# roclark/torchsr

Measured on AMD Instinct MI355X. Metric: 96x96 HR crops/sec (SRGAN GAN train step), higher is better.
Workload: dtype f32; 1 GPU; SRGAN full GAN step (Generator + Discriminator + VGG19 perceptual loss), 96x96 HR crops, batch 16 per GPU, fp32; per_gpu_batch=16, global_batch=16, crop=96, parallelism=dp1, hip_graph=True, vgg19_weights=seeded-random, plan_cus=256

## Files before the change

### include/srx.h

```cpp
#ifndef SRX_H
#define SRX_H

#include <stddef.h>
#include <stdint.h>

#ifdef __cplusplus
extern "C" {
#endif

#define SRX_VERSION 100

enum {
  SRX_OK = 0,
  SRX_E_BADARG = 1,
  SRX_E_UNSUPPORTED = 2,
  SRX_E_HIP = 3,
  SRX_E_WORKSPACE = 4
};

enum { SRX_ACT_NONE = 0, SRX_ACT_RELU = 1, SRX_ACT_LRELU = 2, SRX_ACT_PRELU = 3 };

int srx_version(void);
int srx_last_error(char* buf, size_t n);
int srx_build_info(char* buf, size_t n);
// ... 237 lines not shown
int srx_l1_fwd_count(const float* a, const float* b, float* loss, int64_t n, int64_t count, float* ws, void* stream);
int srx_l1_bwd_count(const float* a, const float* b, const float* gscale, float* da, float* db, int64_t n, int64_t count,
                     void* stream);
int srx_bce_fwd(const float* p, float target, float* loss, int64_t n, float* ws, void* stream);
int srx_bce_bwd(const float* p, float target, const float* gscale, float* dp, int64_t n, void* stream);
int srx_bce_logits_fwd(const float* x, const float* shift, float target, float* loss, int64_t n, float* ws, void* stream);
int srx_bce_logits_bwd(const float* x, const float* shift, float target, const float* gscale, float* dx, int64_t n, void* stream);
int srx_mean_fwd(const float* x, float* out, int64_t n, float* ws, void* stream);
int srx_mean_bwd(const float* x, const float* gscale, float* dx, int64_t n, void* stream);

enum { SRX_HEAD_SRGAN_D = 0, SRX_HEAD_SRGAN_G = 1, SRX_HEAD_ESRGAN_D = 2, SRX_HEAD_ESRGAN_G = 3 };
typedef struct {
  int32_t mode, B, J, n_first;
  float slope, adv_weight;
} srx_gan_head_t;
int srx_gan_head_fwd(const srx_gan_head_t* h, const float* hidden, const float* w2, const float* b2, const float* shift,
                     const float* addend, float* zp, float* out, float* loss, void* stream);
int srx_gan_head_bwd(const srx_gan_head_t* h, const float* hidden, const float* w2, const float* zp, const float* out,
                     const float* shift, const float* g, float* dpre, float* dw2, float* db2, float* db1, int accumulate,
                     void* stream);

int srx_adam_step(float* p, const float* g, float* m, float* v, int64_t n, const float* lr, float beta1,
                  float beta2, float eps, float grad_scale, int64_t* step, void* stream);

#ifdef __cplusplus
}
#endif
#endif
```

### torchsr_amd/_lib.py

```python
import ctypes as C
import os
import subprocess
import sys

_HERE = os.path.dirname(os.path.abspath(__file__))
CSRC = os.path.join(_HERE, 'csrc')
LIB_PATH = os.environ.get('SRX_LIB') or os.path.join(CSRC, 'libsrx_hip.so')
SOURCES = ['api.cpp', 'gconv.hip', 'wgrad.hip', 'convpack.hip', 'c64.hip', 'thin9.hip', 'rdb.hip', 'thin.hip', 'rowtile.hip', 'augment.hip', 'norm.hip', 'eltwise.hip', 'linear.hip', 'loss.hip', 'head.hip', 'wino.hip', 'optim.hip']
HEADERS = ['srx_common.h', 'conv_host.h', os.path.join('..', '..', 'include', 'srx.h')]

ACT_NONE, ACT_RELU, ACT_LRELU, ACT_PRELU = 0, 1, 2, 3


class Conv2dDesc(C.Structure):
    _fields_ = [
        ('N', C.c_int32), ('H', C.c_int32), ('W', C.c_int32),
        ('Cin', C.c_int32), ('Cin_s', C.c_int32), ('Cout', C.c_int32), ('Cout_s', C.c_int32),
        ('KH', C.c_int32), ('KW', C.c_int32), ('stride', C.c_int32), ('pad', C.c_int32),
        ('shuffle', C.c_int32), ('act', C.c_int32), ('slope', C.c_float), ('up', C.c_int32),
        ('precision', C.c_int32),
    ]


class DgradEpilogue(C.Structure):
# ... 220 lines not shown
    'srx_wino_ws_floats': (_Z, [_D, _I]),
    'srx_wino_plan': (_I, [_D, _I, C.POINTER(C.c_int)]),
    'srx_wino_pack': (_I, [_D, _P, _P, _I, _P]),
    'srx_wino_fwd': (_I, [_D, _P, _P, _P, _P, _P, _Z, _P]),
    'srx_wino_bwd_data': (_I, [_D, _P, _P, _P, _P, _P, _Z, _P]),
    'srx_conv3x3_bf16s_applicable': (_I, [_D]),
    'srx_conv3x3_bf16s_packed_bytes': (_Z, [_D]),
    'srx_conv3x3_bf16s_pack': (_I, [_D, _P, _P, _P, _P]),
    'srx_conv3x3_bf16s_ws_floats': (_Z, [_D, _I]),
    'srx_conv3x3_bf16s_fwd': (_I, [_D, _P, _P, _P, _I, _P, _I, _P, _Z, _P]),
    'srx_conv3x3_bf16s_bwd_data': (_I, [_D, _P, _P, _P, _P, _I, _P, _Z, _P]),
    'srx_conv2d_fwd_first3_to_bf16': (_I, [_D, _P, _P, _P, _P, _P]),
    'srx_maxpool2x2_fwd_to_bf16': (_I, [_P, _P, _I, _I, _I, _I, _P]),
    'srx_maxpool2x2_relu_bwd_bf16': (_I, [_P, _P, _P, _I, _I, _I, _I, _P]),
    'srx_act_bwd_from_out_to_bf16': (_I, [_P, _P, _P, C.c_int64, _I, C.c_float, _P]),
    'srx_wino_infer_applicable': (_I, [_D]),
    'srx_wino_fwd_act': (_I, [_D, _P, _P, _P, _P, _P, _P, _Z, _P]),
    'srx_wino_force_plan': (_I, [_I, _I, _I]),
    'srx_wino_stat_rows': (_I, [_D]),
    'srx_wino_fwd_stats': (_I, [_D, _P, _P, _P, _P, _P, _P, _Z, _P]),
    'srx_gan_head_fwd': (_I, [C.POINTER(GanHead), _P, _P, _P, _P, _P, _P, _P, _P, _P]),
    'srx_gan_head_bwd': (_I, [C.POINTER(GanHead), _P, _P, _P, _P, _P, _P, _P, _P, _P, _P, _I, _P]),
    'srx_adam_step': (_I, [_P, _P, _P, _P, _L, _P, _F, _F, _F, _F, _P, _P]),
}
_UNCHECKED = {'srx_wino_applicable', 'srx_wino_infer_applicable', 'srx_conv3x3_bf16s_applicable', 'srx_wino_stat_rows', 'srx_conv2d_bwd_data_bn_rows', 'srx_conv2d_fwd_bn_in_ok', 'srx_conv2d_bwd_data_bn_in_ok', 'srx_pack_table_bytes', 'srx_version', 'srx_last_error', 'srx_device_cus', 'srx_plan_cus', 'srx_prof_stop', 'srx_conv2d_stat_rows', 'srx_bn_stat_rows', 'srx_bn_rows_per_block'}

EXPORTS = tuple(_SIGS.keys())

_lib = None


def load_handle(path: str) -> C.CDLL:
    import torch
    if torch.cuda.is_available():
        torch.cuda.init()
    return C.CDLL(path)


def _ensure_fresh():
    want = source_digest()
    if built_digest(LIB_PATH) == want:
        return
    import fcntl
    with open(os.path.join(CSRC, '.build.lock'), 'w') as lock:
        fcntl.flock(lock, fcntl.LOCK_EX)
        if built_digest(LIB_PATH) == want:
# ... 47 lines not shown
```

### torchsr_amd/csrc/linear.hip

```cpp
#include "srx_common.h"
#include <algorithm>

namespace {

template <int NB>
__global__ __launch_bounds__(256) void linear_fwd_kernel(const float* __restrict__ x, const float* __restrict__ w,
                                                         float* __restrict__ part, int B, int K, int J, int b0,
                                                         int kper) {
  __shared__ f32x4 red[4][64];
  const int tid = threadIdx.x, lane = tid & 63, wave = tid >> 6;
  const int r = lane & 15, h = lane >> 4;
  const int j0 = blockIdx.x * 16;
  const int kbeg = blockIdx.y * kper, kend = min(K, kbeg + kper);
  const int j = j0 + r;
  const bool jok = j < J;
  const float* wr = w + (size_t)(jok ? j : 0) * K;
  const float* xr[NB];
  bool bok[NB];
  f32x4 acc[NB];
#pragma unroll
  for (int n = 0; n < NB; ++n) {
    const int b = b0 + 16 * n + r;
    bok[n] = b < B;
    xr[n] = x + (size_t)(bok[n] ? b : 0) * K;
// ... 322 lines not shown
  f32x4 prev[4];
  if (accumulate) {
#pragma unroll
    for (int g = 0; g < 4; ++g) prev[g] = *reinterpret_cast<const f32x4*>(dw + (size_t)(j0 + 4 * h + g) * K + kcol);
  }
  for (int bb0 = 0; bb0 < B; bb0 += 32) {
    float av[8];
    f32x4 xf[8];
#pragma unroll
    for (int i = 0; i < 8; ++i) {
      av[i] = srx_bload1(rd, dv, (unsigned)srx_uniform((bb0 + 4 * i) * J * 4));
      xf[i] = srx_bload(rx, xv, (unsigned)srx_uniform((bb0 + 4 * i) * K * 4));
    }
#pragma unroll
    for (int i = 0; i < 8; ++i)
#pragma unroll
      for (int e = 0; e < 4; ++e) acc[e] = __builtin_amdgcn_mfma_f32_16x16x4f32(av[i], xf[i][e], acc[e], 0, 0, 0);
  }
#pragma unroll
  for (int g = 0; g < 4; ++g) {
    f32x4 o = {acc[0][g], acc[1][g], acc[2][g], acc[3][g]};
    if (accumulate) o += prev[g];
    *reinterpret_cast<f32x4*>(dw + (size_t)(j0 + 4 * h + g) * K + kcol) = o;
  }
}

bool linear_fast_ok(int B, int K, int J, bool need_j16) {
  const size_t lim = 0xfffffff0ull;
  return K % 64 == 0 && (!need_j16 || J % 16 == 0) && ((size_t)J + 16) * K * 4 < lim && ((size_t)B + 64) * K * 4 < lim && ((size_t)B + 64) * J * 4 < lim;
}

int fwd_splits(int K, int J, int B) {
  const int64_t tiles = srx_cdiv(J, 16) * srx_cdiv(B, 64);
  int64_t s = srx_cdiv(1024, tiles);
  const int64_t maxs = srx_cdiv(K, 256);
  if (s > maxs) s = maxs;
  if (s < 1) s = 1;
  return (int)s;
}
int bwd_splits(int K, int J, int B) {
  const int64_t blocks = srx_cdiv(K, 256) * srx_cdiv(B, 64);
  int64_t s = srx_cdiv(1024, blocks);
  const int64_t maxs = srx_cdiv(J, 64);
  if (s > maxs) s = maxs;
  if (s < 1) s = 1;
  return (int)s;
// ... 56 lines not shown
    else if (nb == 3) hipLaunchKernelGGL(linear_bwd_data_kernel<3>, grid, dim3(256), 0, st, dy, w, ws, B, K, J, b0, jper);
    else hipLaunchKernelGGL(linear_bwd_data_kernel<4>, grid, dim3(256), 0, st, dy, w, ws, B, K, J, b0, jper);
    SRX_CHECK_LAUNCH("linear_bwd_data_kernel");
  }
  const int64_t n = (int64_t)B * K;
  hipLaunchKernelGGL(sum_slabs_kernel, dim3((unsigned)srx_cdiv(n / 4, 256)), dim3(256), 0, st, ws, nsplit, n, dx);
  SRX_CHECK_LAUNCH("sum_slabs_kernel");
  return SRX_OK;
}

extern "C" int srx_linear_bwd_weight(const float* x, const float* dy, float* dw, int accumulate, int B, int K, int J,
                                     void* stream) {
  SRX_REQUIRE(x && dy && dw && B > 0 && K > 0 && J > 0, "linear_bwd_weight: bad argument");
  SRX_REQUIRE(K % 4 == 0, "linear_bwd_weight: in_features must be a multiple of 4");
  if (linear_fast_ok(B, K, J, true))
    hipLaunchKernelGGL(linear_bwd_weight_fast_kernel, dim3((unsigned)srx_cdiv(K, 256), (unsigned)srx_cdiv(J, 16)), dim3(256),
                       0, srx_stream(stream), x, dy, dw, B, K, J, accumulate);
  else
    hipLaunchKernelGGL(linear_bwd_weight_kernel, dim3((unsigned)srx_cdiv(K, 256), (unsigned)srx_cdiv(J, 16)), dim3(256),
                       0, srx_stream(stream), x, dy, dw, B, K, J, accumulate);
  SRX_CHECK_LAUNCH("linear_bwd_weight_kernel");
  return SRX_OK;
}
```

### torchsr_amd/csrc/optim.hip

```cpp
#include "srx_common.h"

namespace {

__global__ void adam_tick_kernel(int64_t* step) { *step += 1; }

__global__ __launch_bounds__(256) void adam_kernel(float* __restrict__ p, const float* __restrict__ g,
                                                   float* __restrict__ m, float* __restrict__ v, int64_t n,
                                                   const float* __restrict__ lr_ptr, float beta1, float beta2,
                                                   float eps, float gscale, const int64_t* __restrict__ step_ptr) {
  const double t = (double)(*step_ptr);
  const float bc1 = (float)(1.0 - pow((double)beta1, t));
  const float bc2 = (float)(1.0 - pow((double)beta2, t));
  const float step_size = lr_ptr[0] / bc1;
  const float bc2_sqrt = sqrtf(bc2);
  const int64_t n4 = n / 4;
  for (int64_t i = (int64_t)blockIdx.x * blockDim.x + threadIdx.x; i < n4; i += (int64_t)gridDim.x * blockDim.x) {
    f32x4 pv = *reinterpret_cast<const f32x4*>(p + i * 4);
    f32x4 gv = *reinterpret_cast<const f32x4*>(g + i * 4);
    f32x4 mv = *reinterpret_cast<const f32x4*>(m + i * 4);
    f32x4 vv = *reinterpret_cast<const f32x4*>(v + i * 4);
#pragma unroll
    for (int e = 0; e < 4; ++e) {
      const float gg = gv[e] * gscale;
      mv[e] = beta1 * mv[e] + (1.f - beta1) * gg;
      vv[e] = beta2 * vv[e] + (1.f - beta2) * gg * gg;
      const float denom = sqrtf(vv[e]) / bc2_sqrt + eps;
      pv[e] -= step_size * (mv[e] / denom);
    }
    *reinterpret_cast<f32x4*>(p + i * 4) = pv;
    *reinterpret_cast<f32x4*>(m + i * 4) = mv;
    *reinterpret_cast<f32x4*>(v + i * 4) = vv;
  }
  if (blockIdx.x == 0 && threadIdx.x < (n & 3)) {
    const int64_t i = n4 * 4 + threadIdx.x;
    const float gg = g[i] * gscale;
    const float mm = beta1 * m[i] + (1.f - beta1) * gg;
    const float vv = beta2 * v[i] + (1.f - beta2) * gg * gg;
    m[i] = mm;
    v[i] = vv;
    p[i] -= step_size * (mm / (sqrtf(vv) / bc2_sqrt + eps));
  }
}

}

extern "C" int srx_adam_step(float* p, const float* g, float* m, float* v, int64_t n, const float* lr, float beta1,
                             float beta2, float eps, float grad_scale, int64_t* step, void* stream) {
  SRX_REQUIRE(p && g && m && v && lr && step && n > 0, "adam_step: bad argument");
  SRX_REQUIRE(((uintptr_t)p % 16 == 0) && ((uintptr_t)g % 16 == 0) && ((uintptr_t)m % 16 == 0) &&
                  ((uintptr_t)v % 16 == 0),
              "adam_step: buffers must be 16-byte aligned");
  hipStream_t st = srx_stream(stream);
  hipLaunchKernelGGL(adam_tick_kernel, dim3(1), dim3(1), 0, st, step);
  SRX_CHECK_LAUNCH("adam_tick_kernel");
  int64_t blocks = srx_cdiv(n / 4, 256);
  if (blocks > 4096) blocks = 4096;
  if (blocks < 1) blocks = 1;
  hipLaunchKernelGGL(adam_kernel, dim3((unsigned)blocks), dim3(256), 0, st, p, g, m, v, n, lr, beta1, beta2, eps,
                     grad_scale, step);
  SRX_CHECK_LAUNCH("adam_kernel");
  return SRX_OK;
}
```

### torchsr_amd/csrc/srx_common.h

```cpp
#pragma once
#include <hip/hip_runtime.h>
#include <hip/hip_ext.h>
#include <stdint.h>
#include <stddef.h>
#include "../../include/srx.h"

typedef float f32x4 __attribute__((ext_vector_type(4)));
typedef float f32x16 __attribute__((ext_vector_type(16)));

void srx_set_error(const char* fmt, ...);

#define SRX_FAIL(code, ...)      \
  do {                           \
    srx_set_error(__VA_ARGS__);  \
    return (code);               \
  } while (0)

#define SRX_REQUIRE(cond, ...) \
  do {                         \
    if (!(cond)) SRX_FAIL(SRX_E_BADARG, __VA_ARGS__); \
  } while (0)

#define SRX_CHECK_LAUNCH(name)                                                        \
  do {                                                                                \
// ... 51 lines not shown
static inline int64_t srx_roundup(int64_t a, int64_t b) { return srx_cdiv(a, b) * b; }

__device__ __forceinline__ void srx_divmod(int m, int d, float inv_d, int& q, int& r) {
  q = __float2int_rz(__int2float_rn(m) * inv_d);
  r = m - q * d;
  if (r < 0) { q -= 1; r += d; }
  if (r >= d) { q += 1; r -= d; }
}

__device__ __forceinline__ __amdgpu_buffer_rsrc_t srx_rsrc(const void* p, unsigned bytes) {
  return __builtin_amdgcn_make_buffer_rsrc(const_cast<void*>(p), (short)0, (int)bytes, 0x00020000);
}
__device__ __forceinline__ f32x4 srx_bload(__amdgpu_buffer_rsrc_t r, unsigned voff, unsigned soff) {
  return __builtin_bit_cast(f32x4, __builtin_amdgcn_raw_buffer_load_b128(r, (int)voff, (int)soff, 0));
}
__device__ __forceinline__ int srx_uniform(int v) { return __builtin_amdgcn_readfirstlane(v); }

__device__ __forceinline__ float srx_wave_sum(float v) {
#pragma unroll
  for (int o = 32; o > 0; o >>= 1) v += __shfl_xor(v, o, 64);
  return v;
}

__device__ __forceinline__ void srx_wino_pack_one(const float* __restrict__ w, float* __restrict__ upk, int Cout, int Cin,
                                                  int transpose, int64_t idx) {
  const int R = transpose == 1 ? Cin : Cout, K = transpose == 1 ? Cout : Cin;
  const int r = (int)(idx / K), k = (int)(idx - (int64_t)r * K);
  const int rsrc = transpose == 2 ? (r % (Cout / 4)) * 4 + r / (Cout / 4) : r;
  float g[3][3];
#pragma unroll
  for (int i = 0; i < 3; ++i)
#pragma unroll
    for (int j = 0; j < 3; ++j)
      g[i][j] = transpose == 1 ? w[(((size_t)k * Cin + r) * 3 + (2 - i)) * 3 + (2 - j)] : w[(((size_t)rsrc * Cin + k) * 3 + i) * 3 + j];
  float t[4][3];
#pragma unroll
  for (int j = 0; j < 3; ++j) {
    t[0][j] = g[0][j];
    t[1][j] = 0.5f * (g[0][j] + g[1][j] + g[2][j]);
    t[2][j] = 0.5f * (g[0][j] - g[1][j] + g[2][j]);
    t[3][j] = g[2][j];
  }
  const int nch = K / 32, rt = R / 32;
  const int jg = r >> 5, mrow = r & 31, kc = k / 32, kk = k % 32, quad = kk >> 2, e = kk & 3, s = quad >> 1, hh = quad & 1;
#pragma unroll
  for (int i = 0; i < 4; ++i) {
// ... 9 lines not shown
```

### torchsr_amd/ddp.py

```python
from typing import Dict, List, Optional, Sequence, Tuple

import torch
import torch.distributed as dist
from torch import Tensor


class BackwardCuts:

    def __init__(self, names: Sequence[str] = ()):
        self.names = set(names)
        self.pairs: Dict[str, List[Tuple[Tensor, Tensor]]] = {}

    def __call__(self, name: str, t: Tensor) -> Tensor:
        if name not in self.names or not torch.is_grad_enabled() or not t.requires_grad:
            return t
        leaf = t.detach().requires_grad_(True)
        self.pairs.setdefault(name, []).append((t, leaf))
        return leaf

    def pending(self, name: str) -> bool:
        return bool(self.pairs.get(name))

    def resume(self, name: str) -> None:
        pairs = [(t, leaf) for t, leaf in self.pairs.pop(name, []) if leaf.grad is not None]
        if pairs:
            torch.autograd.backward([t for t, _ in pairs], [leaf.grad for _, leaf in pairs])

    def clear(self) -> None:
        self.pairs.clear()


class GradBuckets:

    window_bytes = 8 << 20

    def __init__(self, flat, boundaries: Sequence[str] = (), module: Optional[torch.nn.Module] = None,
                 group: Optional[dist.ProcessGroup] = None, force: bool = False, reserve_cus: int = 0, window_hook=None):
        self.reserve_cus = int(reserve_cus)
        self.window_hook = window_hook
        self._window = False
        self.flat = flat
        self.group = group
        self.world_size = dist.get_world_size(group) if dist.is_initialized() else 1
        self.force = bool(force) and dist.is_initialized()
        cuts = [0]
        if boundaries:
            if module is None:
                raise RuntimeError('GradBuckets: boundaries are parameter names of `module`')
            offs = flat.offsets_by_name(module)
            for name in boundaries:
                if name not in offs:
                    raise RuntimeError(f'GradBuckets: no trainable parameter {name!r}')
                cuts.append(offs[name])
        cuts.append(flat.numel)
        if sorted(cuts) != cuts or len(set(cuts)) != len(cuts):
            raise RuntimeError(f'GradBuckets: boundaries must be distinct and in parameter order, got offsets {cuts}')
        self.slices = [flat.grad[a:b] for a, b in zip(cuts[:-1], cuts[1:])]
        self._work = []
        self.issued = 0
        self.timing = False
        self._marks = []
        self._launched = []

    def __len__(self) -> int:
# ... 107 lines not shown
```

### torchsr_amd/esrgan/trainer.py

```python
import torch

from .. import functional as F
from ..layers import no_weight_grad
from ..srgan.trainer import SRGANTrainer
from .discriminator import Discriminator
from .generator import Generator


class ESRGANTrainer(SRGANTrainer):
    phase_prefix = 'esrgan'
    deep_overlap = False
    generator_cls = Generator
    discriminator_cls = Discriminator
    amp_phases = ('psnr', 'gan')
    gen_tail_bucket = 'upsample1.weight'

    def _initialize_loss(self) -> None:
        super()._initialize_loss()
        self.l1_loss = F.l1_loss
        self.pixel_loss = F.l1_loss
        self.bce_loss = F.bce_with_logits

    def _phase_disc(self) -> None:
        self._phase_disc_gen()
        self._phase_disc_loss()

    def _phase_disc_gen(self) -> None:
        with torch.no_grad():
            low4 = F.to_nhwc(self._static['low_res'], 4)
            self._high4 = F.to_nhwc(self._static['high_res'], 4)
        self.disc_optimizer.zero_grad()
        self._super_res = self.generator.forward_nhwc(low4)

    def _phase_disc_loss(self) -> None:
# ... 23 lines not shown
```

### torchsr_amd/functional.py

```python
import contextlib
from typing import Optional, Tuple

import torch
from torch import Tensor
from torch.autograd import Function

from . import _dev, _lib
from ._lib import (ACT_LRELU, ACT_NONE, ACT_PRELU, ACT_RELU, HEAD_ESRGAN_D, HEAD_ESRGAN_G, HEAD_SRGAN_D, HEAD_SRGAN_G,
                   Conv2dDesc, call)

import ctypes as C


direct_grads = [False]


def _sink(param: Optional[Tensor]) -> Optional[Tensor]:
    if not direct_grads[0] or param is None or not param.requires_grad:
        return None
    g = param.grad
    if g is None or not g.is_cuda or g.dtype != torch.float32 or not g.is_contiguous():
        return None
    return g


cut_hook = [None]


def cut_point(name: str, t: Tensor) -> Tensor:
    hook = cut_hook[0]
    return t if hook is None else hook(name, t)


class WeightGradQueue:
    MAXP = 72

    def __init__(self):
        self.groups = {}
        self.pairs = {}

    def add(self, d: Conv2dDesc, x_ptr: int, dy_ptr: int, sink_ptr: int, bias_ptr, keep, scale: float = 1.0) -> None:
        key = tuple(getattr(d, f) for f, _ in Conv2dDesc._fields_)
        self.groups.setdefault(key, [d, []])[1].append((x_ptr, dy_ptr, sink_ptr, bias_ptr or 0, keep, float(scale)))

    def add_pair(self, d: Conv2dDesc, cin_lo: int, x_ptr: int, dy_ptr: int, sinks, bias_sinks, keep) -> None:
        key = ('pair', cin_lo, bias_sinks is None) + tuple(getattr(d, f) for f, _ in Conv2dDesc._fields_)
# ... 1269 lines not shown
        ctx.cfg = (bsz, k, j, act, slope, bias is not None, nws)
        ctx.params = (w, bias)
        ctx.save_for_backward(x, wd, y if act != ACT_NONE else None)
        return y

    @staticmethod
    def backward(ctx, dy: Tensor):
        x, w, y = ctx.saved_tensors
        bsz, k, j, act, slope, has_bias, nws = ctx.cfg
        dy = _chk(dy, 'linear.grad')
        s = _stream()
        if act != ACT_NONE:
            g = torch.empty_like(dy)
            call('srx_act_bwd_from_out', _p(dy), _p(y), _p(g), dy.numel(), act, slope, s)
            dy = g
        dx = dw = db = None
        if ctx.needs_input_grad[0]:
            dx = torch.empty_like(x)
            call('srx_linear_bwd_data', _p(dy), _p(w), _p(dx), bsz, k, j, _p(_ws(nws, x)), nws, s)
        wparam, bparam = ctx.params
        if ctx.needs_input_grad[1]:
            sink = _sink(wparam)
            dw = None if sink is not None else torch.empty_like(w)
            call('srx_linear_bwd_weight', _p(x), _p(dy), _p(dw if sink is None else sink), 0 if sink is None else 1,
                 bsz, k, j, s)
        if has_bias and ctx.needs_input_grad[2]:
            sink = _sink(bparam)
            db = None if sink is not None else torch.empty(j, dtype=torch.float32, device=x.device)
            n2 = _lib.lib().srx_colsum_ws_floats(bsz, j)
            call('srx_colsum', _p(dy), _p(db if sink is None else sink), bsz, j, j, 0 if sink is None else 1,
                 _p(_ws(n2, x)), n2, s)
        return dx, dw, db, None, None


def linear(x: Tensor, w: Tensor, bias: Optional[Tensor], act: int = ACT_NONE, slope: float = 0.0) -> Tensor:
    return _Linear.apply(x, w, bias, act, float(slope))


class _GanHead(Function):

    @staticmethod
    def forward(ctx, x: Tensor, w1: Tensor, b1: Optional[Tensor], w2: Tensor, b2: Optional[Tensor], mode: int, n_first: int,
                slope: float, adv_weight: float, shift: Optional[Tensor], addend: Optional[Tensor]):
        ctx.set_materialize_grads(False)
        x = _chk(x, 'gan_head.input')
        w1d, w2d = _chk(w1.detach(), 'gan_head.weight1'), _chk(w2.detach(), 'gan_head.weight2')
        bsz, k = x.shape
        j = w1d.shape[0]
# ... 34 lines not shown
        direct = all(sk is not None for sk, wnt in zip(sinks, wanted) if wnt) and any(wanted)
        ptrs = [None, None, None, None]
        if not direct:
            if wanted[1]:
                db1 = torch.empty(j, dtype=torch.float32, device=x.device)
            if wanted[2]:
                dw2 = torch.empty_like(w2)
            if wanted[3]:
                db2 = torch.empty(1, dtype=torch.float32, device=x.device)
            ptrs = [None, _p(db1), _p(dw2), _p(db2)]
        else:
            ptrs = [None] + [_p(sk) if wnt else None for sk, wnt in list(zip(sinks, wanted))[1:]]
        dpre = torch.empty((bsz, j), dtype=torch.float32, device=x.device)
        call('srx_gan_head_bwd', C.byref(h), _p(hidden), _p(w2), _p(zp), _p(out), _p(sh), _p(g), _p(dpre), ptrs[2], ptrs[3],
             ptrs[1], 1 if direct else 0, s)
        dx = None
        if need[0]:
            dx = torch.empty_like(x)
            call('srx_linear_bwd_data', _p(dpre), _p(w1), _p(dx), bsz, k, j, _p(_ws(ctx.nws, x)), ctx.nws, s)
        if wanted[0]:
            sink = sinks[0] if direct else None
            if sink is None:
                dw1 = torch.empty_like(w1)
            call('srx_linear_bwd_weight', _p(x), _p(dpre), _p(dw1 if sink is None else sink), 0 if sink is None else 1, bsz, k, j, s)
        dadd = g.view(()) if need[10] else None
        return dx, dw1, db1, (None if dw2 is None else dw2.view_as(w2p)), db2, None, None, None, None, None, dadd


def gan_head(x: Tensor, lin1, lin2, mode: int, n_first: int = 0, slope: float = 0.2, adv_weight: float = 1.0,
             shift: Optional[Tensor] = None, addend: Optional[Tensor] = None):
    from .layers import _w
    return _GanHead.apply(x, _w(lin1.weight), _w(lin1.bias), _w(lin2.weight), _w(lin2.bias), int(mode), int(n_first), float(slope),
                          float(adv_weight), shift, addend)


class _PairLoss(Function):

    @staticmethod
    def forward(ctx, a: Tensor, b: Tensor, kind: str, count: int = 0):
        ctx.set_materialize_grads(False)
        a, b = _chk(a, f'{kind}.input'), _chk(b, f'{kind}.target')
        if a.shape != b.shape:
            raise RuntimeError(f'{kind}_loss: shape mismatch {tuple(a.shape)} vs {tuple(b.shape)}')
        loss = torch.empty((), dtype=torch.float32, device=a.device)
        if count:
            call(f'srx_{kind}_fwd_count', _p(a), _p(b), _p(loss), a.numel(), count, _p(_ws(2048, a)), _stream())
        else:
# ... 663 lines not shown
```

### torchsr_amd/optim.py

```python
from typing import Iterable, List

import torch
from torch import nn, Tensor

from . import functional as F
from ._lib import call


class FlatParams:

    ALIGN = 4

    def __init__(self, module: nn.Module):
        params = [p for p in module.parameters() if p.requires_grad]
        if not params:
            raise RuntimeError('FlatParams: module has no trainable parameters')
        dev, dt = params[0].device, params[0].dtype
        if dt != torch.float32:
            raise RuntimeError('FlatParams: fp32 parameters expected')
        offs, total = [], 0
        for p in params:
            offs.append(total)
            total += (p.numel() + self.ALIGN - 1) // self.ALIGN * self.ALIGN
        self.data = torch.zeros(total, dtype=dt, device=dev)
        self.grad = torch.zeros(total, dtype=dt, device=dev)
        self.params: List[nn.Parameter] = params
        self.offsets: List[int] = offs
        self.numel = total
        self.pack_epoch = [0]
        for m in module.modules():
            st = getattr(m, '_st', None)
            if isinstance(st, F.ConvState):
                st.model_epoch = self.pack_epoch
        with torch.no_grad():
            for p, o in zip(params, offs):
                n = p.numel()
                self.data[o:o + n].copy_(p.detach().reshape(-1))
                p.data = self.data[o:o + n].view(p.shape)
                p.grad = self.grad[o:o + n].view(p.shape)

    def offsets_by_name(self, module: nn.Module) -> dict:
        where = {id(p): o for p, o in zip(self.params, self.offsets)}
        return {n: where[id(p)] for n, p in module.named_parameters() if id(p) in where}

    def zero_grad(self) -> None:
        self.grad.zero_()
        off = 0
        for p in self.params:
            n = p.numel()
            if p.grad is None or p.grad.data_ptr() != self.grad.data_ptr() + off * 4:
                p.grad = self.grad[off:off + n].view(p.shape)
            off += (n + self.ALIGN - 1) // self.ALIGN * self.ALIGN


class FlatAdam:

    def __init__(self, flat: FlatParams, lr: float = 1e-4, betas=(0.9, 0.999), eps: float = 1e-8):
        self.flat = flat
        self.betas, self.eps = betas, eps
        dev = flat.data.device
        self.exp_avg = torch.zeros_like(flat.data)
        self.exp_avg_sq = torch.zeros_like(flat.data)
        self.step_count = torch.zeros((), dtype=torch.int64, device=dev)
        self.lr_dev = torch.tensor(float(lr), dtype=torch.float32, device=dev)
        self._lr = float(lr)
        self.grad_scale = 1.0
        self.pack_table = None
        self.param_groups = [{'lr': float(lr), 'initial_lr': float(lr)}]

    @property
    def lr(self) -> float:
        return self._lr

    def set_lr(self, lr: float) -> None:
        self._lr = float(lr)
        self.param_groups[0]['lr'] = float(lr)
        self.lr_dev.fill_(float(lr))

    def zero_grad(self) -> None:
        self.flat.zero_grad()

    @torch.no_grad()
    def step(self) -> None:
        f = self.flat
        call('srx_adam_step', f.data.data_ptr(), f.grad.data_ptr(), self.exp_avg.data_ptr(),
             self.exp_avg_sq.data_ptr(), f.numel, self.lr_dev.data_ptr(), self.betas[0], self.betas[1], self.eps,
             self.grad_scale, self.step_count.data_ptr(), torch.cuda.current_stream().cuda_stream)
        self.flat.pack_epoch[0] += 1
        if self.pack_table is not None:
            self.pack_table.run()

    def state_dict(self):
        return {'exp_avg': self.exp_avg, 'exp_avg_sq': self.exp_avg_sq, 'step': self.step_count, 'lr': self._lr}

    def load_state_dict(self, sd) -> None:
        self.exp_avg.copy_(sd['exp_avg'])
        self.exp_avg_sq.copy_(sd['exp_avg_sq'])
        self.step_count.copy_(sd['step'])
        self.set_lr(sd['lr'])


class StepLR:

    def __init__(self, optimizer: FlatAdam, step_size: int, gamma: float = 0.1):
        self.optimizer, self.step_size, self.gamma = optimizer, max(1, int(step_size)), gamma
        self.base_lr = optimizer.lr
        self.last_epoch = 0

    def step(self) -> None:
        self.last_epoch += 1
# ... 12 lines not shown
```

### torchsr_amd/srgan/trainer.py

```python
import os
import time
from argparse import Namespace
from math import log10
from typing import Callable, Dict, Optional

import torch
import torch.distributed as dist
from torch import Tensor

from .. import _dev
from .. import functional as F
from ..ddp import BackwardCuts, GradBuckets, broadcast_module
from ..layers import no_weight_grad, set_conv_precision
from ..optim import FlatAdam, FlatParams, StepLR
from .discriminator import Discriminator
from .generator import Generator
from .loss import VGGLoss

try:
    import wandb
except ImportError:
    wandb = None


# ... 45 lines not shown
            self.pushed = count
        if count - min(index) > self.cap:
            raise RuntimeError(f'LossRing: a pending sample is {count - min(index)} records old in a ring of {self.cap} slots '
                               '(flush when note() says so)')
        self.unnoted += (count - self.read) - n
        values = host[:self.cap * 4].view(self.cap, 4)[:, 0]
        for (key, step, contents, _), idx in zip(self.pending, index):
            log({**contents, key: float(values[idx % self.cap])}, step=step)
        self.read = count
        self.pending = []


class SRGANTrainer:

    phase_prefix = 'srgan'
    deep_overlap = True
    overlap_branches = True
    generator_cls = Generator
    discriminator_cls = Discriminator
    amp_phases = ('psnr',)
    gen_tail_bucket = 'conv_layers.0.conv.weight'
    disc_head_bucket = 'classifier.0.weight'
    wandb_flush_every = 50

    def __init__(self, device, args: Namespace, train_loader, test_loader, train_len: int, test_len: int,
                 distributed: bool = False) -> None:
        self.amp = not args.disable_amp
        self.batch_size = args.batch_size
        self.best_psnr = -1.0
        self.device = torch.device(device)
        self.distributed = distributed
        self.epochs = args.epochs
        self.gan_checkpoint = args.gan_checkpoint
        self.local_rank = args.local_rank
        self.pre_epochs = args.pretrain_epochs
        self.psnr_checkpoint = args.psnr_checkpoint
        self.save_image = not args.skip_image_save
        self.test_loader = test_loader
        self.test_len = test_len
        self.train_loader = train_loader
        self.train_len = train_len
        self.world_size = args.world_size
        self.main_process = args.rank in [-1, 0]
        self.use_graphs = bool(getattr(args, 'use_graphs', True))
        self.vgg_weights = getattr(args, 'vgg_weights', None)
        self.force_collectives = bool(getattr(args, 'force_collectives', False))
# ... 40 lines not shown
        self.generator = self.generator_cls().to(self.device)
        self.discriminator = self.discriminator_cls().to(self.device)
        if self.distributed:
            broadcast_module(self.generator)
            broadcast_module(self.discriminator)
        self.gen_flat = FlatParams(self.generator)
        self.disc_flat = FlatParams(self.discriminator)
        force = self.force_collectives
        kw = {'force': force, 'reserve_cus': self.comm_reserved_cus, 'window_hook': self.comm_window_hook}
        self.gen_sync = GradBuckets(self.gen_flat, (self.gen_tail_bucket,), self.generator, **kw) if self.distributed else None
        self.disc_sync = GradBuckets(self.disc_flat, (self.disc_head_bucket,), self.discriminator, **kw) \
            if self.distributed else None

    def _initialize_loss(self) -> None:
        self.mse_loss = F.mse_loss
        self.pixel_loss = F.mse_loss
        self.bce_loss = F.bce_loss
        self.vgg_loss = VGGLoss(weights=self.vgg_weights).to(self.device)

    def _initialize_optimizers(self) -> None:
        self.psnr_optimizer = FlatAdam(self.gen_flat, lr=0.0001, betas=(0.9, 0.999))
        self.disc_optimizer = FlatAdam(self.disc_flat, lr=0.0001, betas=(0.9, 0.999))
        self.gen_optimizer = FlatAdam(self.gen_flat, lr=0.0001, betas=(0.9, 0.999))
        if self.distributed:
            for opt in (self.psnr_optimizer, self.gen_optimizer):
                opt.grad_scale = self.gen_sync.scale
            self.disc_optimizer.grad_scale = self.disc_sync.scale
        from ..layers import Conv2d
        gen_table = F.PackTable(m for m in self.generator.modules() if isinstance(m, Conv2d))
        disc_table = F.PackTable(m for m in self.discriminator.modules() if isinstance(m, Conv2d))
        self.psnr_optimizer.pack_table = self.gen_optimizer.pack_table = gen_table
        self.disc_optimizer.pack_table = disc_table
        self.disc_scheduler = StepLR(self.disc_optimizer, step_size=self.epochs // 8, gamma=0.6)
        self.gen_scheduler = StepLR(self.gen_optimizer, step_size=self.epochs // 8, gamma=0.6)

    def _create_test_image(self) -> None:
        path = 'media/waterfalls-low-res.png'
        if os.path.exists(path):
            import numpy as np
            from PIL import Image
            a = np.asarray(Image.open(path).convert('RGB'), dtype='float32') / 255.0
            image = torch.from_numpy(a).permute(2, 0, 1).contiguous()
        else:
            yy, xx = torch.meshgrid(torch.linspace(0, 1, 320), torch.linspace(0, 1, 480), indexing='ij')
            image = torch.stack([xx, yy, 0.5 + 0.5 * torch.sin(12 * xx * yy)])
        self.test_image = image.unsqueeze(0).to(self.device)
# ... 408 lines not shown
```

Baseline: 2420 crops/s.

## Fuse discriminator classifier weight-gradient GEMM with its Adam update

Defers the discriminator's first classifier Linear weight gradient during graph capture and computes it in a kernel that applies the Adam update directly. The flat Adam pass skips that slice and zero_grad no longer clears it. This avoids writing, zeroing and rereading the large classifier weight gradient. The cost is extra bookkeeping: version checks, single-writer assumptions, and a path that is active only when capturing and not bucketed.

```diff
diff --git a/include/srx.h b/include/srx.h
--- a/include/srx.h
+++ b/include/srx.h
@@ -283,6 +283,11 @@
 
 int srx_adam_step(float* p, const float* g, float* m, float* v, int64_t n, const float* lr, float beta1,
                   float beta2, float eps, float grad_scale, int64_t* step, void* stream);
+int srx_adam_step_skip(float* p, const float* g, float* m, float* v, int64_t n, int64_t skip_begin, int64_t skip_count,
+                       const float* lr, float beta1, float beta2, float eps, float grad_scale, int64_t* step, void* stream);
+int srx_linear_bwd_weight_adam(const float* x, const float* dy, float* p, float* m, float* v, int B, int K, int J,
+                               const float* lr, float beta1, float beta2, float eps, float grad_scale, const int64_t* step,
+                               void* stream);
 
 #ifdef __cplusplus
 }
diff --git a/torchsr_amd/_lib.py b/torchsr_amd/_lib.py
--- a/torchsr_amd/_lib.py
+++ b/torchsr_amd/_lib.py
@@ -266,6 +266,8 @@
     'srx_gan_head_fwd': (_I, [C.POINTER(GanHead), _P, _P, _P, _P, _P, _P, _P, _P, _P]),
     'srx_gan_head_bwd': (_I, [C.POINTER(GanHead), _P, _P, _P, _P, _P, _P, _P, _P, _P, _P, _I, _P]),
     'srx_adam_step': (_I, [_P, _P, _P, _P, _L, _P, _F, _F, _F, _F, _P, _P]),
+    'srx_adam_step_skip': (_I, [_P, _P, _P, _P, _L, _L, _L, _P, _F, _F, _F, _F, _P, _P]),
+    'srx_linear_bwd_weight_adam': (_I, [_P, _P, _P, _P, _P, _I, _I, _I, _P, _F, _F, _F, _F, _P, _P]),
 }
 _UNCHECKED = {'srx_wino_applicable', 'srx_wino_infer_applicable', 'srx_conv3x3_bf16s_applicable', 'srx_wino_stat_rows', 'srx_conv2d_bwd_data_bn_rows', 'srx_conv2d_fwd_bn_in_ok', 'srx_conv2d_bwd_data_bn_in_ok', 'srx_pack_table_bytes', 'srx_version', 'srx_last_error', 'srx_device_cus', 'srx_plan_cus', 'srx_prof_stop', 'srx_conv2d_stat_rows', 'srx_bn_stat_rows', 'srx_bn_rows_per_block'}
 
diff --git a/torchsr_amd/csrc/linear.hip b/torchsr_amd/csrc/linear.hip
--- a/torchsr_amd/csrc/linear.hip
+++ b/torchsr_amd/csrc/linear.hip
@@ -368,6 +368,80 @@
     f32x4 o = {acc[0][g], acc[1][g], acc[2][g], acc[3][g]};
     if (accumulate) o += prev[g];
     *reinterpret_cast<f32x4*>(dw + (size_t)(j0 + 4 * h + g) * K + kcol) = o;
+  }
+}
+
+template <bool FAST>
+__global__ __launch_bounds__(256) void linear_bwd_weight_adam_kernel(const float* __restrict__ x, const float* __restrict__ dy,
+                                                                     float* __restrict__ p, float* __restrict__ m,
+                                                                     float* __restrict__ v, int B, int K, int J,
+                                                                     const float* __restrict__ lr_ptr, float beta1, float beta2,
+                                                                     float eps, float gscale, const int64_t* __restrict__ step_ptr) {
+  const int tid = threadIdx.x, lane = tid & 63, wave = srx_uniform(tid >> 6);
+  const int r = lane & 15, h = lane >> 4;
+  const int n0 = (blockIdx.x * 4 + wave) * 64;
+  if (n0 >= K) return;
+  const int j0 = blockIdx.y * 16;
+  const int kcol = n0 + 4 * r;
+  const bool kok = kcol < K;
+  f32x4 pv[4], mv[4], vv[4];
+  bool ok[4];
+#pragma unroll
+  for (int g = 0; g < 4; ++g) {
+    const int jj = j0 + 4 * h + g;
+    ok[g] = FAST || (kok && jj < J);
+    const size_t at = ok[g] ? (size_t)jj * K + kcol : 0;
+    pv[g] = *reinterpret_cast<const f32x4*>(p + at);
+    mv[g] = *reinterpret_cast<const f32x4*>(m + at);
+    vv[g] = *reinterpret_cast<const f32x4*>(v + at);
+  }
+  f32x4 acc[4];
+#pragma unroll
+  for (int e = 0; e < 4; ++e) acc[e] = (f32x4){0.f, 0.f, 0.f, 0.f};
+  if constexpr (FAST) {
+    const __amdgpu_buffer_rsrc_t rx = srx_rsrc(x, (unsigned)((size_t)B * K * 4)), rd = srx_rsrc(dy, (unsigned)((size_t)B * J * 4));
+    const unsigned xv = 4u * ((unsigned)h * (unsigned)K + (unsigned)kcol), dv = 4u * ((unsigned)h * (unsigned)J + (unsigned)(j0 + r));
+    for (int bb0 = 0; bb0 < B; bb0 += 32) {
+      float av[8];
+      f32x4 xf[8];
+#pragma unroll
+      for (int i = 0; i < 8; ++i) {
+        av[i] = srx_bload1(rd, dv, (unsigned)srx_uniform((bb0 + 4 * i) * J * 4));
+        xf[i] = srx_bload(rx, xv, (unsigned)srx_uniform((bb0 + 4 * i) * K * 4));
+      }
+#pragma unroll
+      for (int i = 0; i < 8; ++i)
+#pragma unroll
+        for (int e = 0; e < 4; ++e) acc[e] = __builtin_amdgcn_mfma_f32_16x16x4f32(av[i], xf[i][e], acc[e], 0, 0, 0);
+    }
+  } else {
+    const int j = j0 + r;
+    const bool jok = j < J;
+    for (int bb = 0; bb < B; bb += 4) {
+      const int b = bb + h;
+      const bool bok = b < B;
+      const float a = dy[(size_t)(bok ? b : 0) * J + (jok ? j : 0)];
+      const float av = (bok && jok) ? a : 0.f;
+      const f32x4 xl = *reinterpret_cast<const f32x4*>(x + (size_t)(bok ? b : 0) * K + (kok ? kcol : 0));
+      const f32x4 xv = (bok && kok) ? xl : (f32x4){0.f, 0.f, 0.f, 0.f};
+#pragma unroll
+      for (int e = 0; e < 4; ++e) acc[e] = __builtin_amdgcn_mfma_f32_16x16x4f32(av, xv[e], acc[e], 0, 0, 0);
+    }
+  }
+  const srx_adam_coef_t c = srx_adam_coef(lr_ptr, beta1, beta2, step_ptr);
+#pragma unroll
+  for (int g = 0; g < 4; ++g) {
+    if (!ok[g]) continue;
+    const size_t at = (size_t)(j0 + 4 * h + g) * K + kcol;
+#pragma unroll
+    for (int e = 0; e < 4; ++e) {
+      float pe = pv[g][e], me = mv[g][e], ve = vv[g][e];
+      srx_adam_update(pe, me, ve, acc[e][g], gscale, beta1, beta2, eps, c);
+      pv[g][e] = pe, mv[g][e] = me, vv[g][e] = ve;
+    }
+    *reinterpret_cast<f32x4*>(p + at) = pv[g];
+    *reinterpret_cast<f32x4*>(m + at) = mv[g];
+    *reinterpret_cast<f32x4*>(v + at) = vv[g];
   }
 }
 
@@ -470,3 +544,21 @@
   SRX_CHECK_LAUNCH("linear_bwd_weight_kernel");
   return SRX_OK;
 }
+
+extern "C" int srx_linear_bwd_weight_adam(const float* x, const float* dy, float* p, float* m, float* v, int B, int K, int J,
+                                          const float* lr, float beta1, float beta2, float eps, float grad_scale,
+                                          const int64_t* step, void* stream) {
+  SRX_REQUIRE(x && dy && p && m && v && lr && step && B > 0 && K > 0 && J > 0, "linear_bwd_weight_adam: bad argument");
+  SRX_REQUIRE(K % 4 == 0, "linear_bwd_weight_adam: in_features must be a multiple of 4");
+  SRX_REQUIRE(((uintptr_t)x % 16 == 0) && ((uintptr_t)p % 16 == 0) && ((uintptr_t)m % 16 == 0) && ((uintptr_t)v % 16 == 0),
+              "linear_bwd_weight_adam: x, p, m, v must be 16-byte aligned");
+  const dim3 grid((unsigned)srx_cdiv(K, 256), (unsigned)srx_cdiv(J, 16));
+  if (linear_fast_ok(B, K, J, true))
+    hipLaunchKernelGGL(linear_bwd_weight_adam_kernel<true>, grid, dim3(256), 0, srx_stream(stream), x, dy, p, m, v, B, K, J, lr,
+                       beta1, beta2, eps, grad_scale, step);
+  else
+    hipLaunchKernelGGL(linear_bwd_weight_adam_kernel<false>, grid, dim3(256), 0, srx_stream(stream), x, dy, p, m, v, B, K, J, lr,
+                       beta1, beta2, eps, grad_scale, step);
+  SRX_CHECK_LAUNCH("linear_bwd_weight_adam_kernel");
+  return SRX_OK;
+}
diff --git a/torchsr_amd/csrc/optim.hip b/torchsr_amd/csrc/optim.hip
--- a/torchsr_amd/csrc/optim.hip
+++ b/torchsr_amd/csrc/optim.hip
@@ -4,60 +4,75 @@
 
 __global__ void adam_tick_kernel(int64_t* step) { *step += 1; }
 
+template <bool SKIP>
 __global__ __launch_bounds__(256) void adam_kernel(float* __restrict__ p, const float* __restrict__ g,
                                                    float* __restrict__ m, float* __restrict__ v, int64_t n,
                                                    const float* __restrict__ lr_ptr, float beta1, float beta2,
-                                                   float eps, float gscale, const int64_t* __restrict__ step_ptr) {
-  const double t = (double)(*step_ptr);
-  const float bc1 = (float)(1.0 - pow((double)beta1, t));
-  const float bc2 = (float)(1.0 - pow((double)beta2, t));
-  const float step_size = lr_ptr[0] / bc1;
-  const float bc2_sqrt = sqrtf(bc2);
-  const int64_t n4 = n / 4;
+                                                   float eps, float gscale, const int64_t* __restrict__ step_ptr,
+                                                   int64_t skip4_begin, int64_t skip4_len) {
+  const srx_adam_coef_t c = srx_adam_coef(lr_ptr, beta1, beta2, step_ptr);
+  const int64_t n4 = n / 4 - (SKIP ? skip4_len : 0);
   for (int64_t i = (int64_t)blockIdx.x * blockDim.x + threadIdx.x; i < n4; i += (int64_t)gridDim.x * blockDim.x) {
-    f32x4 pv = *reinterpret_cast<const f32x4*>(p + i * 4);
-    f32x4 gv = *reinterpret_cast<const f32x4*>(g + i * 4);
-    f32x4 mv = *reinterpret_cast<const f32x4*>(m + i * 4);
-    f32x4 vv = *reinterpret_cast<const f32x4*>(v + i * 4);
+    const int64_t q = (SKIP && i >= skip4_begin) ? i + skip4_len : i;
+    f32x4 pv = *reinterpret_cast<const f32x4*>(p + q * 4);
+    f32x4 gv = *reinterpret_cast<const f32x4*>(g + q * 4);
+    f32x4 mv = *reinterpret_cast<const f32x4*>(m + q * 4);
+    f32x4 vv = *reinterpret_cast<const f32x4*>(v + q * 4);
 #pragma unroll
     for (int e = 0; e < 4; ++e) {
-      const float gg = gv[e] * gscale;
-      mv[e] = beta1 * mv[e] + (1.f - beta1) * gg;
-      vv[e] = beta2 * vv[e] + (1.f - beta2) * gg * gg;
-      const float denom = sqrtf(vv[e]) / bc2_sqrt + eps;
-      pv[e] -= step_size * (mv[e] / denom);
+      float pe = pv[e], me = mv[e], ve = vv[e];
+      srx_adam_update(pe, me, ve, gv[e], gscale, beta1, beta2, eps, c);
+      pv[e] = pe, mv[e] = me, vv[e] = ve;
     }
-    *reinterpret_cast<f32x4*>(p + i * 4) = pv;
-    *reinterpret_cast<f32x4*>(m + i * 4) = mv;
-    *reinterpret_cast<f32x4*>(v + i * 4) = vv;
+    *reinterpret_cast<f32x4*>(p + q * 4) = pv;
+    *reinterpret_cast<f32x4*>(m + q * 4) = mv;
+    *reinterpret_cast<f32x4*>(v + q * 4) = vv;
   }
   if (blockIdx.x == 0 && threadIdx.x < (n & 3)) {
-    const int64_t i = n4 * 4 + threadIdx.x;
-    const float gg = g[i] * gscale;
-    const float mm = beta1 * m[i] + (1.f - beta1) * gg;
-    const float vv = beta2 * v[i] + (1.f - beta2) * gg * gg;
+    const int64_t i = (n / 4) * 4 + threadIdx.x;
+    float pp = p[i], mm = m[i], vv = v[i];
+    srx_adam_update(pp, mm, vv, g[i], gscale, beta1, beta2, eps, c);
     m[i] = mm;
     v[i] = vv;
-    p[i] -= step_size * (mm / (sqrtf(vv) / bc2_sqrt + eps));
+    p[i] = pp;
   }
+}
+
+int adam_launch(float* p, const float* g, float* m, float* v, int64_t n, int64_t skip_begin, int64_t skip_count, const float* lr,
+                float beta1, float beta2, float eps, float grad_scale, int64_t* step, void* stream) {
+  SRX_REQUIRE(p && g && m && v && lr && step && n > 0, "adam_step: bad argument");
+  SRX_REQUIRE(((uintptr_t)p % 16 == 0) && ((uintptr_t)g % 16 == 0) && ((uintptr_t)m % 16 == 0) &&
+                  ((uintptr_t)v % 16 == 0),
+              "adam_step: buffers must be 16-byte aligned");
+  SRX_REQUIRE(skip_begin >= 0 && skip_count >= 0 && skip_begin % 4 == 0 && skip_count % 4 == 0 && skip_begin <= n &&
+                  skip_count <= n - skip_begin,
+              "adam_step: the skipped range must be whole float4s inside the buffer");
+  hipStream_t st = srx_stream(stream);
+  hipLaunchKernelGGL(adam_tick_kernel, dim3(1), dim3(1), 0, st, step);
+  SRX_CHECK_LAUNCH("adam_tick_kernel");
+  if (n - skip_count <= 0) return SRX_OK;
+  int64_t blocks = srx_cdiv((n - skip_count) / 4, 256);
+  if (blocks > 4096) blocks = 4096;
+  if (blocks < 1) blocks = 1;
+  if (skip_count)
+    hipLaunchKernelGGL(adam_kernel<true>, dim3((unsigned)blocks), dim3(256), 0, st, p, g, m, v, n, lr, beta1, beta2, eps,
+                       grad_scale, step, skip_begin / 4, skip_count / 4);
+  else
+    hipLaunchKernelGGL(adam_kernel<false>, dim3((unsigned)blocks), dim3(256), 0, st, p, g, m, v, n, lr, beta1, beta2, eps,
+                       grad_scale, step, (int64_t)0, (int64_t)0);
+  SRX_CHECK_LAUNCH("adam_kernel");
+  return SRX_OK;
 }
 
 }
 
 extern "C" int srx_adam_step(float* p, const float* g, float* m, float* v, int64_t n, const float* lr, float beta1,
                              float beta2, float eps, float grad_scale, int64_t* step, void* stream) {
-  SRX_REQUIRE(p && g && m && v && lr && step && n > 0, "adam_step: bad argument");
-  SRX_REQUIRE(((uintptr_t)p % 16 == 0) && ((uintptr_t)g % 16 == 0) && ((uintptr_t)m % 16 == 0) &&
-                  ((uintptr_t)v % 16 == 0),
-              "adam_step: buffers must be 16-byte aligned");
-  hipStream_t st = srx_stream(stream);
-  hipLaunchKernelGGL(adam_tick_kernel, dim3(1), dim3(1), 0, st, step);
-  SRX_CHECK_LAUNCH("adam_tick_kernel");
-  int64_t blocks = srx_cdiv(n / 4, 256);
-  if (blocks > 4096) blocks = 4096;
-  if (blocks < 1) blocks = 1;
-  hipLaunchKernelGGL(adam_kernel, dim3((unsigned)blocks), dim3(256), 0, st, p, g, m, v, n, lr, beta1, beta2, eps,
-                     grad_scale, step);
-  SRX_CHECK_LAUNCH("adam_kernel");
-  return SRX_OK;
+  return adam_launch(p, g, m, v, n, 0, 0, lr, beta1, beta2, eps, grad_scale, step, stream);
 }
+
+extern "C" int srx_adam_step_skip(float* p, const float* g, float* m, float* v, int64_t n, int64_t skip_begin,
+                                  int64_t skip_count, const float* lr, float beta1, float beta2, float eps, float grad_scale,
+                                  int64_t* step, void* stream) {
+  return adam_launch(p, g, m, v, n, skip_begin, skip_count, lr, beta1, beta2, eps, grad_scale, step, stream);
+}
diff --git a/torchsr_amd/csrc/srx_common.h b/torchsr_amd/csrc/srx_common.h
--- a/torchsr_amd/csrc/srx_common.h
+++ b/torchsr_amd/csrc/srx_common.h
@@ -97,6 +97,23 @@
   return v;
 }
 
+struct srx_adam_coef_t { float step_size, bc2_sqrt; };
+__device__ __forceinline__ srx_adam_coef_t srx_adam_coef(const float* lr_ptr, float beta1, float beta2, const int64_t* step_ptr) {
+  const double t = (double)(*step_ptr);
+  const float bc1 = (float)(1.0 - pow((double)beta1, t));
+  const float bc2 = (float)(1.0 - pow((double)beta2, t));
+  return {lr_ptr[0] / bc1, sqrtf(bc2)};
+}
+__device__ __forceinline__ void srx_adam_update(float& p, float& m, float& v, float g, float gscale, float beta1, float beta2,
+                                                float eps, srx_adam_coef_t c) {
+#pragma clang fp contract(off)
+  const float gg = g * gscale;
+  m = __builtin_fmaf(1.f - beta1, gg, beta1 * m);
+  v = __builtin_fmaf(beta2, v, gg * ((1.f - beta2) * gg));
+  const float denom = sqrtf(v) / c.bc2_sqrt + eps;
+  p = __builtin_fmaf(-c.step_size, m / denom, p);
+}
+
 __device__ __forceinline__ void srx_wino_pack_one(const float* __restrict__ w, float* __restrict__ upk, int Cout, int Cin,
                                                   int transpose, int64_t idx) {
   const int R = transpose == 1 ? Cin : Cout, K = transpose == 1 ? Cout : Cin;
diff --git a/torchsr_amd/ddp.py b/torchsr_amd/ddp.py
--- a/torchsr_amd/ddp.py
+++ b/torchsr_amd/ddp.py
@@ -40,6 +40,7 @@
         self.window_hook = window_hook
         self._window = False
         self.flat = flat
+        flat.bucketed = True
         self.group = group
         self.world_size = dist.get_world_size(group) if dist.is_initialized() else 1
         self.force = bool(force) and dist.is_initialized()
diff --git a/torchsr_amd/esrgan/trainer.py b/torchsr_amd/esrgan/trainer.py
--- a/torchsr_amd/esrgan/trainer.py
+++ b/torchsr_amd/esrgan/trainer.py
@@ -10,6 +10,7 @@
 class ESRGANTrainer(SRGANTrainer):
     phase_prefix = 'esrgan'
     deep_overlap = False
+    fuse_classifier_adam = False
     generator_cls = Generator
     discriminator_cls = Discriminator
     amp_phases = ('psnr', 'gan')
diff --git a/torchsr_amd/functional.py b/torchsr_amd/functional.py
--- a/torchsr_amd/functional.py
+++ b/torchsr_amd/functional.py
@@ -22,6 +22,13 @@
     if g is None or not g.is_cuda or g.dtype != torch.float32 or not g.is_contiguous():
         return None
     return g
+
+
+def _linear_bwd_weight(param: Tensor, x: Tensor, dy: Tensor, sink: Tensor, bsz: int, k: int, j: int, s: int) -> None:
+    opt = getattr(param, '_fused_adam', None)
+    if opt is not None and opt.defer_linear_weight(x, dy, bsz, k, j):
+        return
+    call('srx_linear_bwd_weight', _p(x), _p(dy), _p(sink), 1, bsz, k, j, s)
 
 
 cut_hook = [None]
@@ -1337,8 +1344,10 @@
         if ctx.needs_input_grad[1]:
             sink = _sink(wparam)
             dw = None if sink is not None else torch.empty_like(w)
-            call('srx_linear_bwd_weight', _p(x), _p(dy), _p(dw if sink is None else sink), 0 if sink is None else 1,
-                 bsz, k, j, s)
+            if sink is not None:
+                _linear_bwd_weight(wparam, x, dy, sink, bsz, k, j, s)
+            else:
+                call('srx_linear_bwd_weight', _p(x), _p(dy), _p(dw), 0, bsz, k, j, s)
         if has_bias and ctx.needs_input_grad[2]:
             sink = _sink(bparam)
             db = None if sink is not None else torch.empty(j, dtype=torch.float32, device=x.device)
@@ -1419,7 +1428,9 @@
             sink = sinks[0] if direct else None
             if sink is None:
                 dw1 = torch.empty_like(w1)
-            call('srx_linear_bwd_weight', _p(x), _p(dpre), _p(dw1 if sink is None else sink), 0 if sink is None else 1, bsz, k, j, s)
+                call('srx_linear_bwd_weight', _p(x), _p(dpre), _p(dw1), 0, bsz, k, j, s)
+            else:
+                _linear_bwd_weight(w1p, x, dpre, sink, bsz, k, j, s)
         dadd = g.view(()) if need[10] else None
         return dx, dw1, db1, (None if dw2 is None else dw2.view_as(w2p)), db2, None, None, None, None, None, dadd
 
diff --git a/torchsr_amd/optim.py b/torchsr_amd/optim.py
--- a/torchsr_amd/optim.py
+++ b/torchsr_amd/optim.py
@@ -28,6 +28,7 @@
         self.offsets: List[int] = offs
         self.numel = total
         self.pack_epoch = [0]
+        self.bucketed = False
         for m in module.modules():
             st = getattr(m, '_st', None)
             if isinstance(st, F.ConvState):
@@ -43,8 +44,13 @@
         where = {id(p): o for p, o in zip(self.params, self.offsets)}
         return {n: where[id(p)] for n, p in module.named_parameters() if id(p) in where}
 
-    def zero_grad(self) -> None:
-        self.grad.zero_()
+    def zero_grad(self, skip=None) -> None:
+        if skip is None:
+            self.grad.zero_()
+        else:
+            for part in (self.grad[:skip[0]], self.grad[skip[0] + skip[1]:]):
+                if part.numel():
+                    part.zero_()
         off = 0
         for p in self.params:
             n = p.numel()
@@ -66,6 +72,9 @@
         self._lr = float(lr)
         self.grad_scale = 1.0
         self.pack_table = None
+        self._fused = None
+        self._deferred = None
+        self._fused_step = False
         self.param_groups = [{'lr': float(lr), 'initial_lr': float(lr)}]
 
     @property
@@ -77,15 +86,49 @@
         self.param_groups[0]['lr'] = float(lr)
         self.lr_dev.fill_(float(lr))
 
+    def fuse_linear_weight(self, weight: nn.Parameter) -> None:
+        at = [i for i, p in enumerate(self.flat.params) if p is weight]
+        if len(at) != 1 or weight.dim() != 2 or weight.shape[1] % 4 or self.flat.offsets[at[0]] % 4:
+            raise RuntimeError('fuse_linear_weight: a [out, in] weight of this optimiser with in_features % 4 == 0 at a '
+                               '16-byte aligned offset of the flat buffer expected')
+        self._fused = (self.flat.offsets[at[0]], weight.numel(), tuple(weight.shape))
+        weight._fused_adam = self
+
     def zero_grad(self) -> None:
-        self.flat.zero_grad()
+        self._deferred = None
+        self._fused_step = (self._fused is not None and not self.flat.bucketed and torch.cuda.is_current_stream_capturing())
+        self.flat.zero_grad(self._fused[:2] if self._fused_step else None)
+
+    def defer_linear_weight(self, x: Tensor, dy: Tensor, bsz: int, k: int, j: int) -> bool:
+        if not self._fused_step:
+            return False
+        if (j, k) != self._fused[2] or self._deferred is not None:
+            raise RuntimeError('FlatAdam: the fused Linear weight has ONE gradient writer of its own shape per step')
+        self._deferred = (x, dy, bsz, x._version, dy._version)
+        return True
 
     @torch.no_grad()
     def step(self) -> None:
         f = self.flat
-        call('srx_adam_step', f.data.data_ptr(), f.grad.data_ptr(), self.exp_avg.data_ptr(),
-             self.exp_avg_sq.data_ptr(), f.numel, self.lr_dev.data_ptr(), self.betas[0], self.betas[1], self.eps,
-             self.grad_scale, self.step_count.data_ptr(), torch.cuda.current_stream().cuda_stream)
+        s = torch.cuda.current_stream().cuda_stream
+        hyper = (self.lr_dev.data_ptr(), self.betas[0], self.betas[1], self.eps, self.grad_scale)
+        deferred, self._deferred = self._deferred, None
+        fused_step, self._fused_step = self._fused_step, False
+        if not fused_step:
+            call('srx_adam_step', f.data.data_ptr(), f.grad.data_ptr(), self.exp_avg.data_ptr(),
+                 self.exp_avg_sq.data_ptr(), f.numel, *hyper, self.step_count.data_ptr(), s)
+        else:
+            if deferred is None:
+                raise RuntimeError('FlatAdam: the fused Linear weight got no gradient in this step (its slice was not cleared)')
+            x, dy, bsz, xv, dyv = deferred
+            if (x._version, dy._version) != (xv, dyv):
+                raise RuntimeError('FlatAdam: an operand of the deferred Linear weight gradient was modified in place')
+            off, count, (j, k) = self._fused
+            call('srx_adam_step_skip', f.data.data_ptr(), f.grad.data_ptr(), self.exp_avg.data_ptr(),
+                 self.exp_avg_sq.data_ptr(), f.numel, off, count, *hyper, self.step_count.data_ptr(), s)
+            call('srx_linear_bwd_weight_adam', x.data_ptr(), dy.data_ptr(), f.data.data_ptr() + 4 * off,
+                 self.exp_avg.data_ptr() + 4 * off, self.exp_avg_sq.data_ptr() + 4 * off, bsz, k, j, *hyper,
+                 self.step_count.data_ptr(), s)
         self.flat.pack_epoch[0] += 1
         if self.pack_table is not None:
             self.pack_table.run()
diff --git a/torchsr_amd/srgan/trainer.py b/torchsr_amd/srgan/trainer.py
--- a/torchsr_amd/srgan/trainer.py
+++ b/torchsr_amd/srgan/trainer.py
@@ -91,6 +91,7 @@
     gen_tail_bucket = 'conv_layers.0.conv.weight'
     disc_head_bucket = 'classifier.0.weight'
     wandb_flush_every = 50
+    fuse_classifier_adam = True
 
     def __init__(self, device, args: Namespace, train_loader, test_loader, train_len: int, test_len: int,
                  distributed: bool = False) -> None:
@@ -177,6 +178,8 @@
         self.psnr_optimizer = FlatAdam(self.gen_flat, lr=0.0001, betas=(0.9, 0.999))
         self.disc_optimizer = FlatAdam(self.disc_flat, lr=0.0001, betas=(0.9, 0.999))
         self.gen_optimizer = FlatAdam(self.gen_flat, lr=0.0001, betas=(0.9, 0.999))
+        if self.fuse_classifier_adam:
+            self.disc_optimizer.fuse_linear_weight(self.discriminator.classifier[0].weight)
         if self.distributed:
             for opt in (self.psnr_optimizer, self.gen_optimizer):
                 opt.grad_scale = self.gen_sync.scale
```

New measurement: 2437 crops/s (median of 6 runs). About the same (+0.7%).
